# russellgeum/Digging-into-Self-Supervised-Monocular-Depth-Estimation

Hardware: AMD Instinct MI355X
Metric: images/sec training, KITTI 192x640 batch 12/GPU (higher is better)
Workload: dtype f32; 1 GPU; configs[1]: kitti_eigen_zhou-shaped 192x640, batch 12/GPU, ResNet18 depth + separate ResNet18 pose, frame_ids [0,-1,1], 4 scales, automask, Adam, fp32; global_batch=12, parallelism=dp1

## Files before the change

digging-into-self-supervised-monocular-depth-estimation_amd/csrc/thinconv_nhwc.hip:

```cpp
#include "nhwc_common.hpp"

namespace mdx {
namespace nhwc {

typedef float v4f __attribute__((ext_vector_type(4)));
constexpr int TW_WAVES = 4;

template <int CIN>
__global__ __launch_bounds__(64 * TW_WAVES) void thin_wgrad16_kernel(const float *__restrict__ x, const float *__restrict__ gy, int B, int h,
                                                                      int w, int quads_per_wave, float *__restrict__ part)
{
    constexpr int CH = CIN / 16, NT = 9 * CH;
    __shared__ float lds[TW_WAVES][256];
    const int lane = threadIdx.x & 63, wave = threadIdx.x >> 6;
    const int Hp = h + 2, Wp = w + 2, wq = w / 4;
    const long long nquads = (long long)B * h * wq;
    const long long q0 = ((long long)blockIdx.x * TW_WAVES + wave) * quads_per_wave;
    const long long q1 = q0 + quads_per_wave < nquads ? q0 + quads_per_wave : nquads;
    v4f acc[NT];
#pragma unroll
    for (int t = 0; t < NT; ++t) acc[t] = (v4f){0.f, 0.f, 0.f, 0.f};
    const int k = lane >> 4, j = lane & 15;
    if (q0 < q1) {
        int qx = (int)(q0 % wq);
        const long long row0 = q0 / wq;
        int i = (int)(row0 % h);
        const int b0 = (int)(row0 / h);
        const float *pg = gy + (size_t)q0 * 64 + lane;
        const float *px = x + (((size_t)b0 * Hp + i) * Wp + (size_t)qx * 4 + k) * CIN + j;
        auto load_b = [&](const float *xb, float (&bv)[NT]) {
#pragma unroll
            for (int ty = 0; ty < 3; ++ty)
#pragma unroll
                for (int tx = 0; tx < 3; ++tx)
#pragma unroll
                    for (int c = 0; c < CH; ++c) bv[(ty * 3 + tx) * CH + c] = xb[((size_t)ty * Wp + tx) * CIN + c * 16];
        };
        auto advance = [&]() {
            pg += 64;
            px += 4 * CIN;
            if (++qx == wq) {
                qx = 0;
                px += 2 * CIN;
                if (++i == h) { i = 0; px += (size_t)2 * Wp * CIN; }
            }
        };
        float a0 = *pg, b0v[NT];
        load_b(px, b0v);
        for (long long q = q0; q < q1; ++q) {
            float a1 = 0.f, b1v[NT];
            advance();
            if (q + 1 < q1) {
                a1 = *pg;
                load_b(px, b1v);
            } else {
#pragma unroll
                for (int t = 0; t < NT; ++t) b1v[t] = 0.f;
            }
#pragma unroll
            for (int t = 0; t < NT; ++t) acc[t] = __builtin_amdgcn_mfma_f32_16x16x4f32(a0, b0v[t], acc[t], 0, 0, 0);
            a0 = a1;
#pragma unroll
            for (int t = 0; t < NT; ++t) b0v[t] = b1v[t];
        }
    }
    float *dst = part + (size_t)blockIdx.x * NT * 256;
#pragma unroll
    for (int t = 0; t < NT; ++t) {
#pragma unroll
        for (int v = 0; v < 4; ++v) lds[wave][(4 * k + v) * 16 + j] = acc[t][v];
        __syncthreads();
        {
            const int r = threadIdx.x;
            float s = lds[0][r];
#pragma unroll
            for (int u = 1; u < TW_WAVES; ++u) s += lds[u][r];
            dst[t * 256 + r] = s;
        }
        __syncthreads();
    }
}

constexpr int TF_S = 64;
__global__ __launch_bounds__(16 * TF_S) void thin_wgrad16_finish_kernel(const float *__restrict__ part, int nblk, int CIN, long wso, long wsc,
                                                                        long wsy, long wsx, float *__restrict__ gw)
{
    __shared__ float lds[TF_S / 4][16];
    const int n = 9 * CIN * 16;
    const int cl = threadIdx.x % 16, sl = threadIdx.x / 16, e = blockIdx.x * 16 + cl;
    float s = 0.f;
    for (int i = sl; i < nblk; i += TF_S) s += (e < n) ? part[(size_t)i * n + e] : 0.f;
    s += __shfl_down(s, 32, 64);
    s += __shfl_down(s, 16, 64);
    if ((threadIdx.x & 63) < 16) lds[threadIdx.x >> 6][cl] = s;
    __syncthreads();
    if (threadIdx.x < 16 && e < n) {
        float tot = 0.f;
#pragma unroll
        for (int u = 0; u < TF_S / 4; ++u) tot += lds[u][cl];
        const int CH = CIN / 16;
        const int t = e >> 8, r = e & 255, co = r >> 4, cj = r & 15;
        const int tap = t / CH, ci = (t % CH) * 16 + cj;
        gw[co * wso + ci * wsc + (tap / 3) * wsy + (tap % 3) * wsx] = tot;
    }
}

struct ThinGeom { int blocks, quads_per_wave; };
static inline ThinGeom thin_geom(int B, int h, int w)
{
    const long long nquads = (long long)B * h * (w / 4);
    ThinGeom g;
    long long waves = 6144;
    if (waves * 48 > nquads) waves = (nquads + 47) / 48;
    if (waves < 1) waves = 1;
    g.quads_per_wave = (int)((nquads + waves - 1) / waves);
    g.blocks = (int)((nquads + (long long)g.quads_per_wave * TW_WAVES - 1) / ((long long)g.quads_per_wave * TW_WAVES));
    return g;
}

}
}

using namespace mdx;
using namespace mdx::nhwc;

static int thin_args_ok(int B, int Cin, int Cout, int h, int w)
{
    if (B <= 0 || h <= 0 || w <= 0 || w % 4 || Cout != 16 || (Cin != 16 && Cin != 32)) return MDX_ERR_BAD_SHAPE;
    if ((long long)B * (h + 2) * (w + 2) * Cin >= (1ll << 40)) return MDX_ERR_BAD_SHAPE;
    return MDX_OK;
}

MDX_EXPORT size_t mdx_thin_conv3x3_wgrad_workspace_bytes(int B, int Cin, int Cout, int h, int w)
{
    if (thin_args_ok(B, Cin, Cout, h, w)) return 0;
    return (size_t)thin_geom(B, h, w).blocks * 9 * Cin * 16 * sizeof(float);
}

MDX_EXPORT int mdx_thin_conv3x3_wgrad(const float *x, const float *gy, float *gweight, int64_t s_o, int64_t s_c, int64_t s_y, int64_t s_x,
                                      int B, int Cin, int Cout, int h, int w, void *workspace, size_t workspace_bytes, void *stream)
{
    if (!x || !gy || !gweight || !workspace) return MDX_ERR_NULL_POINTER;
    const int bad = thin_args_ok(B, Cin, Cout, h, w);
    if (bad) return bad;
    if (workspace_bytes < mdx_thin_conv3x3_wgrad_workspace_bytes(B, Cin, Cout, h, w)) return MDX_ERR_WORKSPACE;
    const ThinGeom g = thin_geom(B, h, w);
    float *part = (float *)workspace;
    hipStream_t st = (hipStream_t)stream;
    if (Cin == 16)
        hipLaunchKernelGGL((thin_wgrad16_kernel<16>), dim3(g.blocks), dim3(64 * TW_WAVES), 0, st, x, gy, B, h, w, g.quads_per_wave, part);
    else
        hipLaunchKernelGGL((thin_wgrad16_kernel<32>), dim3(g.blocks), dim3(64 * TW_WAVES), 0, st, x, gy, B, h, w, g.quads_per_wave, part);
    const int n = 9 * Cin * 16;
    hipLaunchKernelGGL(thin_wgrad16_finish_kernel, dim3((n + 15) / 16), dim3(16 * TF_S), 0, st, part, g.blocks, Cin, (long)s_o, (long)s_c,
                       (long)s_y, (long)s_x, gweight);
    return check_launch();
}
```

digging-into-self-supervised-monocular-depth-estimation_amd/mdx/functional.py:

```python
import ctypes as C

import torch

from . import _lib
from ._lib import api, ptr, stream, workspace


def _f32c(t, keep_format=False):
    if t is not None and t.dtype != torch.float32:
        t = t.float()
    if t is None or t.is_contiguous() or (keep_format and t.is_contiguous(memory_format=torch.channels_last)):
        return t
    return t.contiguous()


def _byref(struct):
    return C.byref(struct) if struct is not None else None


class _ComposeProjection(torch.autograd.Function):
    @staticmethod
    def forward(ctx, K, T):
        K, T = _f32c(K), _f32c(T)
        B = K.shape[0]
# ... 467 lines not shown
        cam, P = ctx.saved_tensors
        B, H, W, eps = ctx.dims
        ggrid = _f32c(ggrid)
        gcam = torch.empty_like(cam)
        gP = torch.empty_like(P)
        nws = api.mdx_project_workspace_bytes(B, H, W)
        ws = workspace(nws, cam.device)
        api.mdx_project_bwd(ptr(cam), ptr(P), ptr(ggrid), B, H, W, eps, ptr(gcam), ptr(gP),
                            ptr(ws, torch.uint8), nws, stream())
        return gcam, gP, None, None, None


def project(cam, P, H, W, eps=1e-7):
    return _Project.apply(cam, P, int(H), int(W), float(eps))


class _GridSampleBorder(torch.autograd.Function):
    @staticmethod
    def forward(ctx, img, grid):
        img, grid = _f32c(img), _f32c(grid)
        B, Cc, Hi, Wi = img.shape
        _, Ho, Wo, _ = grid.shape
        out = torch.empty(B, Cc, Ho, Wo, device=img.device, dtype=torch.float32)
        api.mdx_grid_sample_border_fwd(ptr(img), ptr(grid), B, Cc, Hi, Wi, Ho, Wo, ptr(out), stream())
        ctx.save_for_backward(img, grid)
        return out

    @staticmethod
    def backward(ctx, gout):
        img, grid = ctx.saved_tensors
        B, Cc, Hi, Wi = img.shape
        _, Ho, Wo, _ = grid.shape
        gout = _f32c(gout)
        ggrid = torch.empty_like(grid)
        gimg = torch.empty_like(img) if ctx.needs_input_grad[0] else None
        api.mdx_grid_sample_border_bwd(ptr(img), ptr(grid), ptr(gout), B, Cc, Hi, Wi, Ho, Wo, ptr(ggrid),
                                       ptr(gimg, optional=True), stream())
        return gimg, ggrid


def grid_sample_border(img, grid):
    return _GridSampleBorder.apply(img, grid)


class _ReprojectionLoss(torch.autograd.Function):
    @staticmethod
    def forward(ctx, pred, target):
        pred, target = _f32c(pred), _f32c(target)
        B, _, H, W = pred.shape
        out = torch.empty(B, 1, H, W, device=pred.device, dtype=torch.float32)
        api.mdx_reprojection_loss_fwd(ptr(pred), ptr(target), B, H, W, ptr(out), stream())
        ctx.save_for_backward(pred, target)
        return out

    @staticmethod
    def backward(ctx, gout):
        pred, target = ctx.saved_tensors
        B, _, H, W = pred.shape
        gout = _f32c(gout)
        gp = torch.empty_like(pred) if ctx.needs_input_grad[0] else None
        gt = torch.empty_like(pred) if ctx.needs_input_grad[1] else None
        if gp is None and gt is None:
            return None, None
        api.mdx_reprojection_loss_bwd(ptr(pred), ptr(target), ptr(gout), B, H, W, ptr(gp, optional=True),
                                      ptr(gt, optional=True), stream())
        return gp, gt


def reprojection_loss(pred, target):
    return _ReprojectionLoss.apply(pred, target)


class _Ssim(torch.autograd.Function):
    @staticmethod
    def forward(ctx, x, y):
        x, y = _f32c(x), _f32c(y)
        B, Cc, H, W = x.shape
        out = torch.empty_like(x)
        api.mdx_ssim_fwd(ptr(x), ptr(y), B * Cc, H, W, ptr(out), stream())
        ctx.save_for_backward(x, y)
        return out

    @staticmethod
    def backward(ctx, gout):
        x, y = ctx.saved_tensors
        B, Cc, H, W = x.shape
        gout = _f32c(gout)
        gx = torch.empty_like(x) if ctx.needs_input_grad[0] else None
        gy = torch.empty_like(x) if ctx.needs_input_grad[1] else None
        if gx is None and gy is None:
            return None, None
        api.mdx_ssim_bwd(ptr(x), ptr(y), ptr(gout), B * Cc, H, W, ptr(gx, optional=True), ptr(gy, optional=True),
                         stream())
        return gx, gy


def ssim(x, y):
    return _Ssim.apply(x, y)


def min_automask(ident, noise, reproj, automask=True, need_combined=False):
    reproj = _f32c(reproj)
    B, S, H, W = reproj.shape
    dev = reproj.device
    if automask:
        ident, noise = _f32c(ident), _f32c(noise)
    Cc = 2 * S if automask else S
    comb = torch.empty(B, Cc, H, W, device=dev, dtype=torch.float32) if need_combined else None
    to_opt = torch.empty(B, H, W, device=dev, dtype=torch.float32)
    idx = torch.empty(B, H, W, device=dev, dtype=torch.uint8)
    api.mdx_min_automask_fwd(ptr(ident, optional=True) if automask else None,
                             ptr(noise, optional=True) if automask else None, ptr(reproj), B, S, H, W,
                             int(automask), ptr(comb, optional=True), ptr(to_opt), ptr(idx, torch.uint8), stream())
    return to_opt, idx, comb


_DTYPE_CODE = {torch.float32: 0, torch.bfloat16: 1}
_CL = torch.channels_last


from .layout import is_channels_last


def _nhwc_ok(dtype, *channels):
    n = 4 if dtype == torch.float32 else 8
    return all(c % n == 0 for c in channels)


def _layout(x, what, *channels):
    if not x.is_cuda:
        raise _lib.MdxError("%s needs CUDA tensors (the HIP path has no CPU fallback), got %s" % (what, x.device))
    if x.dtype not in _DTYPE_CODE:
        raise _lib.MdxError("%s supports float32 / bfloat16, got %s" % (what, x.dtype))
    cl = is_channels_last(x) and _nhwc_ok(x.dtype, *channels)
    return _DTYPE_CODE[x.dtype], cl, (_CL if cl else torch.contiguous_format)


def _as(t, cl):
    if t is None:
        return None
    return t.contiguous(memory_format=_CL) if cl else t.contiguous()


def _cl_map(x, dtypes=_DTYPE_CODE):
    return x.is_cuda and x.dim() == 4 and x.dtype in dtypes and is_channels_last(x)


class _DecoderGlue(torch.autograd.Function):
    @staticmethod
    def forward(ctx, raw, skip, bias, elu, upsample, out_dtype):
        B, C1, h, w = raw.shape
        u = 2 if upsample else 1
        C2 = 0
        if skip is not None:
            if skip.dtype != raw.dtype or skip.shape[0] != B or tuple(skip.shape[2:]) != (u * h, u * w):
                raise _lib.MdxError("decoder_glue: skip %s %s does not match raw %s %s (x%d)"
                                    % (tuple(skip.shape), skip.dtype, tuple(raw.shape), raw.dtype, u))
            C2 = skip.shape[1]
        in_code, cl, fmt = _layout(raw, "decoder_glue", C1, C2)
        raw, skip, bias = _as(raw, cl), _as(skip, cl), _f32c(bias)
        if bias is not None and bias.shape != (C1,):
            raise _lib.MdxError("decoder_glue: bias %s for %d channels" % (tuple(bias.shape), C1))
        out = torch.empty(B, C1 + C2, u * h + 2, u * w + 2, device=raw.device, dtype=out_dtype, memory_format=fmt)
        fn = api.mdx_decoder_glue_nhwc_fwd if cl else api.mdx_decoder_glue_fwd
        fn(ptr(raw, raw.dtype, cl=cl), ptr(skip, raw.dtype, optional=True, cl=cl), ptr(bias, optional=True),
           ptr(out, out_dtype, cl=cl), B, C1, C2, h, w, int(upsample), int(elu), in_code, _DTYPE_CODE[out_dtype], stream())
        ctx.save_for_backward(raw, bias)
        ctx.meta = (C2, bool(elu), bool(upsample), out_dtype, cl, fmt)
        return out

    @staticmethod
    def backward(ctx, gout):
        raw, bias = ctx.saved_tensors
        C2, elu, upsample, out_dtype, cl, fmt = ctx.meta
        B, C1, h, w = raw.shape
        u = 2 if upsample else 1
        gout = _as(gout.to(out_dtype), cl)
        graw = torch.empty_like(raw)
        gskip = torch.empty(B, C2, u * h, u * w, device=raw.device, dtype=raw.dtype, memory_format=fmt) if C2 else None
        dbias = ws = None
        nws = 0
        code = _DTYPE_CODE[raw.dtype]
        if bias is not None:
            dbias = torch.empty(C1, device=raw.device, dtype=torch.float32)
            nws = (api.mdx_decoder_glue_nhwc_workspace_bytes(B, C1, h, w, code) if cl
                   else api.mdx_decoder_glue_workspace_bytes(B, C1, h, w))
            ws = workspace(nws, raw.device)
        fn = api.mdx_decoder_glue_nhwc_bwd if cl else api.mdx_decoder_glue_bwd
        fn(ptr(gout, out_dtype, cl=cl), ptr(raw, raw.dtype, cl=cl), ptr(bias, optional=True), ptr(graw, raw.dtype, cl=cl),
           ptr(gskip, raw.dtype, optional=True, cl=cl), ptr(dbias, optional=True), B, C1, C2, h, w, int(upsample), int(elu), code,
           _DTYPE_CODE[out_dtype], ptr(ws, torch.uint8, optional=True), nws, stream())
        return graw, gskip, dbias, None, None, None


def decoder_glue(raw, skip=None, elu=True, upsample=True, out_dtype=None, bias=None):
    out_dtype = out_dtype or raw.dtype
    if skip is not None and skip.dtype != raw.dtype:
        skip = skip.to(raw.dtype)
    return _DecoderGlue.apply(raw, skip, bias, bool(elu), bool(upsample), out_dtype)


class _BiasAct(torch.autograd.Function):
    @staticmethod
    def forward(ctx, x, bias, relu):
        B, Cc, H, W = x.shape
        x = _as(x, True)
        y = torch.empty_like(x)
        api.mdx_bias_act_nhwc_fwd(ptr(x, x.dtype, cl=True), ptr(_f32c(bias)), ptr(y, x.dtype, cl=True), B, Cc, H, W, int(relu),
                                  _DTYPE_CODE[x.dtype], stream())
        ctx.save_for_backward(y)
        ctx.meta = (bool(relu), bias.dtype)
        return y

    @staticmethod
    def backward(ctx, dy):
        (y,) = ctx.saved_tensors
        relu, bdt = ctx.meta
        B, Cc, H, W = y.shape
        code = _DTYPE_CODE[y.dtype]
        dy = _as(dy.to(y.dtype), True)
        dx = torch.empty_like(y)
        db = torch.empty(Cc, device=y.device, dtype=torch.float32)
        nws = api.mdx_bias_act_nhwc_workspace_bytes(B, Cc, H, W, code)
        ws = workspace(nws, y.device)
        api.mdx_bias_act_nhwc_bwd(ptr(dy, y.dtype, cl=True), ptr(y, y.dtype, cl=True), ptr(dx, y.dtype, cl=True), ptr(db), B, Cc,
                                  H, W, int(relu), code, ptr(ws, torch.uint8), nws, stream())
        return dx, db.to(bdt), None


def bias_act_ok(x):
    return _cl_map(x) and _nhwc_ok(x.dtype, x.shape[1])


def bias_act(x, bias, relu=True):
    if not bias_act_ok(x):
        raise _lib.MdxError("bias_act: needs a channels-last GPU map with whole 16-byte channel vectors, got %s %s" % (tuple(x.shape), x.dtype))
    return _BiasAct.apply(x, bias, bool(relu))


class _MeanBias(torch.autograd.Function):
    @staticmethod
    def forward(ctx, x, bias, scale):
        B, Cc, H, W = x.shape
        x = _as(x, True)
        out = torch.empty(B, Cc, device=x.device, dtype=torch.float32)
        api.mdx_mean_bias_nhwc_fwd(ptr(x, x.dtype, cl=True), ptr(_f32c(bias), optional=True), ptr(out), B, Cc, H, W, scale,
                                   _DTYPE_CODE[x.dtype], stream())
        ctx.meta = (tuple(x.shape), x.dtype, float(scale), None if bias is None else bias.dtype)
        return out

    @staticmethod
    def backward(ctx, g):
        (B, Cc, H, W), dt, scale, bdt = ctx.meta
        g = _f32c(g)
        dx = torch.empty((B, Cc, H, W), device=g.device, dtype=dt, memory_format=_CL)
        db = torch.empty(Cc, device=g.device, dtype=torch.float32) if bdt is not None else None
        api.mdx_mean_bias_nhwc_bwd(ptr(g), ptr(dx, dt, cl=True), ptr(db, optional=True), B, Cc, H, W, scale, _DTYPE_CODE[dt],
                                   stream())
        return dx, (db.to(bdt) if db is not None else None), None


def mean_bias_ok(x):
    return _cl_map(x)


def mean_bias(x, bias=None, scale=1.0):
    if not mean_bias_ok(x):
        raise _lib.MdxError("mean_bias: needs a channels-last GPU map, got %s %s" % (tuple(x.shape), x.dtype))
    return _MeanBias.apply(x, bias, float(scale))


class FrameStack(object):

    def __init__(self, blocks):
        self.blocks = [list(b) for b in blocks]

    def tensor(self):
        rows = [torch.cat(b, 1) if len(b) > 1 else b[0] for b in self.blocks]
        return torch.cat(rows, 0) if len(rows) > 1 else rows[0]

    def ok(self):
        fr = [t for b in self.blocks for t in b]
        first = fr[0]
        return (1 <= len(self.blocks) <= 2 and len({len(b) for b in self.blocks}) == 1 and 1 <= len(self.blocks[0]) <= 2
                and all(t.is_cuda and t.dtype == torch.float32 and t.dim() == 4 and t.shape == first.shape and t.shape[1] == 3
                        and t.is_contiguous() and not t.requires_grad for t in fr))


def encoder_input(stack, mean=0.45, std=0.225, dtype=torch.float32):
    if not stack.ok():
        raise _lib.MdxError("encoder_input: needs 1-2 blocks of 1-2 planar float32 [n,3,H,W] GPU frames that require no gradient")
    fr = [t for b in stack.blocks for t in b]
    n, _, H, W = fr[0].shape
    blocks, groups = len(stack.blocks), len(stack.blocks[0])
    out = torch.empty((blocks * n, 3 * groups, H, W), device=fr[0].device, dtype=dtype, memory_format=_CL)
    inv = float(torch.tensor(1.0, dtype=torch.float32) / torch.tensor(std, dtype=torch.float32))
    api.mdx_encoder_input_nhwc(_lib.ptr_array(fr), blocks, groups, n, H, W, mean, inv, ptr(out, dtype, cl=True),
                               _DTYPE_CODE[dtype], stream())
    return out


class _ThinConv3x3(torch.autograd.Function):
    ARGS = ([1, 1], [0, 0], [1, 1], False, [0, 0], 1)

    @staticmethod
    def forward(ctx, x, weight):
        ctx.save_for_backward(x, weight)
        return torch.ops.aten.convolution(x, weight, None, *_ThinConv3x3.ARGS)

    @staticmethod
    def backward(ctx, gy):
        x, weight = ctx.saved_tensors
        gx = gw = None
        if ctx.needs_input_grad[0]:
            gx = torch.ops.aten.convolution_backward(gy, x, weight, None, *_ThinConv3x3.ARGS, [True, False, False])[0]
        if ctx.needs_input_grad[1]:
            B, Cin, Hp, Wp = x.shape
            gy = _as(gy, True)
            gw = torch.empty_like(weight)
            nws = api.mdx_thin_conv3x3_wgrad_workspace_bytes(B, Cin, 16, Hp - 2, Wp - 2)
            ws = workspace(nws, x.device)
            api.mdx_thin_conv3x3_wgrad(ptr(x, cl=True), ptr(gy, cl=True), ptr(gw, cl="any"), gw.stride(0), gw.stride(1),
                                       gw.stride(2), gw.stride(3), B, Cin, 16, Hp - 2, Wp - 2, ptr(ws, torch.uint8), nws, stream())
        return gx, gw


def thin_conv_ok(x, weight):
    return (_cl_map(x, (torch.float32,)) and weight.dtype == torch.float32 and tuple(weight.shape) == (16, x.shape[1], 3, 3)
            and x.shape[1] in (16, 32) and x.shape[3] > 2 and (x.shape[3] - 2) % 4 == 0 and x.shape[2] > 2
            and (weight.is_contiguous() or weight.is_contiguous(memory_format=_CL)) and not torch.is_autocast_enabled())


def thin_conv3x3(x, weight):
    if not thin_conv_ok(x, weight):
        raise _lib.MdxError("thin_conv3x3: needs a float32 channels-last map with 16 or 32 channels and a [16,Cin,3,3] weight, got %s %s"
                            % (tuple(x.shape), tuple(weight.shape)))
    return _ThinConv3x3.apply(x, weight)


class _DispHead(torch.autograd.Function):
    @staticmethod
    def forward(ctx, x, weight, bias):
        B, Cc, Hp, Wp = x.shape
        x = _as(x, True)
        w32 = _f32c(weight, keep_format=True)
        disp = torch.empty(B, 1, Hp - 2, Wp - 2, device=x.device, dtype=torch.float32)
        _, sc, sy, sx = w32.stride()
        api.mdx_disp_head_nhwc_fwd(ptr(x, x.dtype, cl=True), ptr(w32, cl="any"), sc, sy, sx, ptr(_f32c(bias), optional=True),
                                   ptr(disp), B, Cc, Hp - 2, Wp - 2, _DTYPE_CODE[x.dtype], stream())
        ctx.save_for_backward(x, w32, disp)
        ctx.meta = (weight.dtype, None if bias is None else bias.dtype)
        return disp

    @staticmethod
    def backward(ctx, g):
        x, w32, disp = ctx.saved_tensors
        wdt, bdt = ctx.meta
        B, Cc, Hp, Wp = x.shape
        code = _DTYPE_CODE[x.dtype]
        g = _f32c(g)
        gx = torch.empty_like(x)
        gw = torch.empty_like(w32)
        gb = torch.empty(1, device=x.device, dtype=torch.float32) if bdt is not None else None
        nws = api.mdx_disp_head_nhwc_workspace_bytes(B, Cc, Hp - 2, Wp - 2, code)
        ws = workspace(nws, x.device)
        _, sc, sy, sx = w32.stride()
        api.mdx_disp_head_nhwc_bwd(ptr(x, x.dtype, cl=True), ptr(w32, cl="any"), sc, sy, sx, ptr(g), ptr(disp),
                                   ptr(gx, x.dtype, cl=True), ptr(gw, cl="any"), ptr(gb, optional=True), B, Cc,
                                   Hp - 2, Wp - 2, code, ptr(ws, torch.uint8), nws, stream())
        return gx, gw.to(wdt), (gb.to(bdt) if gb is not None else None)


def disp_head_ok(x, weight):
    if not _cl_map(x):
        return False
    n = 4
    lp = x.shape[1] // n
    return (tuple(weight.shape) == (1, x.shape[1], 3, 3) and x.shape[1] % n == 0 and 1 <= lp <= 64 and lp & (lp - 1) == 0
            and x.shape[2] > 2 and x.shape[3] > 2)


def disp_head(x, weight, bias=None):
    if not disp_head_ok(x, weight):
        raise _lib.MdxError("disp_head: needs a channels-last GPU map [B,C,h+2,w+2] with C a power of two from 4 to 256 "
                            "and a [1,C,3,3] weight; got x %s %s, weight %s" % (tuple(x.shape), x.dtype, tuple(weight.shape)))
    return _DispHead.apply(x, weight, bias)


class _MaxPool3s2(torch.autograd.Function):
    @staticmethod
    def forward(ctx, x, fork):
        B, Cc, H, W = x.shape
        code, cl, fmt = _layout(x, "maxpool3s2", Cc)
        x = _as(x, cl)
        Ho, Wo = (H - 1) // 2 + 1, (W - 1) // 2 + 1
        out = torch.empty(B, Cc, Ho, Wo, device=x.device, dtype=x.dtype, memory_format=fmt)
        arg = torch.empty(B, Cc, Ho, Wo, device=x.device, dtype=torch.uint8, memory_format=fmt)
        if cl:
            api.mdx_maxpool3s2_nhwc_fwd(ptr(x, x.dtype, cl=True), ptr(out, x.dtype, cl=True),
                                        ptr(arg, torch.uint8, cl=True), B, Cc, H, W, code, stream())
        else:
            api.mdx_maxpool3s2_fwd(ptr(x, x.dtype), ptr(out, x.dtype), ptr(arg, torch.uint8), B * Cc, H, W, code,
                                   stream())
        ctx.save_for_backward(arg)
        ctx.meta = (H, W, x.dtype, cl, fmt)
        ctx.set_materialize_grads(False)
        return (out, out.view_as(out)) if fork else out

    @staticmethod
    def backward(ctx, gout, gout2=None):
        (arg,) = ctx.saved_tensors
        H, W, dtype, cl, fmt = ctx.meta
        B, Cc = arg.shape[:2]
        gout, gout2 = _two_grads(gout, gout2, dtype, cl, fused_add=cl)
        if gout is None:
            return None, None
        gin = torch.empty(B, Cc, H, W, device=gout.device, dtype=dtype, memory_format=fmt)
        if cl:
            api.mdx_maxpool3s2_nhwc_bwd(ptr(gout, dtype, cl=True), ptr(gout2, dtype, optional=True, cl=True),
                                        ptr(arg, torch.uint8, cl=True), ptr(gin, dtype, cl=True), B, Cc, H, W,
                                        _DTYPE_CODE[dtype], stream())
        else:
            api.mdx_maxpool3s2_bwd(ptr(gout, dtype), ptr(arg, torch.uint8), ptr(gin, dtype), B * Cc, H, W,
                                   _DTYPE_CODE[dtype], stream())
        return gin, None


def _two_grads(g1, g2, dtype, cl, fused_add):
    gs = [_as(g.to(dtype), cl) for g in (g1, g2) if g is not None]
    if not gs:
        return None, None
    if len(gs) == 2 and not fused_add:
        gs = [gs[0] + gs[1]]
    return gs[0], (gs[1] if len(gs) == 2 else None)


def maxpool3s2(x, fork=False):
    return _MaxPool3s2.apply(x, bool(fork))


def _residual(what, res, x):
    if res is not None and (res.shape != x.shape or res.dtype != x.dtype):
        raise _lib.MdxError("%s: residual %s %s does not match x %s %s" % (what, tuple(res.shape), res.dtype, tuple(x.shape), x.dtype))
    return res


class _BnAct(torch.autograd.Function):

    @staticmethod
    def forward(ctx, x, res, weight, bias, running_mean, running_var, eps, momentum, relu, groups, fork):
        B, Cc, H, W = x.shape
        code, cl, _ = _layout(x, "bn_act", Cc)
        if B % groups:
            raise _lib.MdxError("bn_act: batch %d is not divisible into %d groups" % (B, groups))
        x, res = _as(x, cl), _as(_residual("bn_act", res, x), cl)
        weight, bias = _f32c(weight), _f32c(bias)
        y = torch.empty_like(x)
        save_mean = torch.empty(groups, Cc, device=x.device, dtype=torch.float32)
        save_invstd = torch.empty(groups, Cc, device=x.device, dtype=torch.float32)
        Bg = B // groups
        nws = api.mdx_bn_nhwc_workspace_bytes(Bg, Cc, H, W, groups, code) if cl else api.mdx_bn_workspace_bytes(Bg, Cc, H, W)
        ws = workspace(nws, x.device)
        fn = api.mdx_bn_act_nhwc_fwd if cl else api.mdx_bn_act_fwd
        fn(ptr(x, x.dtype, cl=cl), ptr(res, x.dtype, optional=True, cl=cl), ptr(weight), ptr(bias),
           ptr(running_mean, optional=True), ptr(running_var, optional=True), ptr(y, x.dtype, cl=cl), ptr(save_mean),
           ptr(save_invstd), Bg, Cc, H, W, groups, eps, momentum, int(relu), code, ptr(ws, torch.uint8), nws, stream())
        mask_from_x = cl and bool(relu) and res is None and x.dtype == torch.float32
        ctx.save_for_backward(x, bias if mask_from_x else y, weight, save_mean, save_invstd)
        ctx.meta = (bool(relu), res is not None, groups, cl, mask_from_x)
        ctx.mark_non_differentiable(*[t for t in (running_mean, running_var) if t is not None])
        ctx.set_materialize_grads(False)
        return (y, y.view_as(y)) if fork else y

    @staticmethod
    def backward(ctx, dy, dy2=None):
        x, y, weight, save_mean, save_invstd = ctx.saved_tensors
        relu, has_res, groups, cl, mask_from_x = ctx.meta
        bias = None
        if mask_from_x:
            y, bias = None, y
        dy, dy2 = _two_grads(dy, dy2, x.dtype, cl, fused_add=cl)
        if dy is None:
            return (None,) * 11
        B, Cc, H, W = x.shape
        Bg = B // groups
        code = _DTYPE_CODE[x.dtype]
        dx = torch.empty_like(x)
        dres = torch.empty_like(x) if has_res else None
        dgamma = torch.empty(Cc, device=x.device, dtype=torch.float32)
        dbeta = torch.empty(Cc, device=x.device, dtype=torch.float32)
        nws = api.mdx_bn_nhwc_workspace_bytes(Bg, Cc, H, W, groups, code) if cl else api.mdx_bn_workspace_bytes(Bg, Cc, H, W)
        ws = workspace(nws, x.device)
        if cl:
            api.mdx_bn_act_nhwc_bwd(
                ptr(dy, x.dtype, cl=True), ptr(dy2, x.dtype, optional=True, cl=True), ptr(y, x.dtype, optional=True, cl=True),
                ptr(x, x.dtype, cl=True), ptr(weight), ptr(bias, optional=True), ptr(save_mean), ptr(save_invstd),
                ptr(dx, x.dtype, cl=True), ptr(dres, x.dtype, optional=True, cl=True), ptr(dgamma), ptr(dbeta), Bg, Cc, H, W,
                groups, int(relu), code, ptr(ws, torch.uint8), nws, stream())
        else:
            api.mdx_bn_act_bwd(
                ptr(dy, x.dtype), ptr(y, x.dtype), ptr(x, x.dtype), ptr(weight), ptr(save_mean), ptr(save_invstd),
                ptr(dx, x.dtype), ptr(dres, x.dtype, optional=True), ptr(dgamma), ptr(dbeta), Bg, Cc, H, W, groups,
                int(relu), code, ptr(ws, torch.uint8), nws, stream())
        return (dx, dres, dgamma, dbeta) + (None,) * 7


def bn_act(x, weight, bias, running_mean, running_var, eps=1e-5, momentum=0.1, residual=None, relu=True, groups=1,
           fork=False):
    return _BnAct.apply(x, residual, weight, bias, running_mean, running_var, float(eps), float(momentum), bool(relu),
                        int(groups), bool(fork))


def bn_act_infer(x, weight, bias, running_mean, running_var, eps=1e-5, residual=None, relu=True, fork=False):
    B, Cc, H, W = x.shape
    code, cl, _ = _layout(x, "bn_act_infer", Cc)
    x, residual = _as(x, cl), _as(_residual("bn_act_infer", residual, x), cl)
    y = torch.empty_like(x)
    fn = api.mdx_bn_act_nhwc_infer if cl else api.mdx_bn_act_infer
    fn(ptr(x, x.dtype, cl=cl), ptr(residual, x.dtype, optional=True, cl=cl), ptr(_f32c(weight)),
       ptr(_f32c(bias)), ptr(_f32c(running_mean)), ptr(_f32c(running_var)), ptr(y, x.dtype, cl=cl), B, Cc, H, W, float(eps),
       int(bool(relu)), code, stream())
    return (y, y.view_as(y)) if fork else y


class _Param2Matrix(torch.autograd.Function):
    @staticmethod
    def forward(ctx, axisangle, translation, invert):
        aa, tr = _f32c(axisangle).reshape(-1, 3), _f32c(translation).reshape(-1, 3)
        N = aa.shape[0]
        if tr.shape[0] != N:
            raise _lib.MdxError("param2matrix: %d rotations, %d translations" % (N, tr.shape[0]))
        M = torch.empty(N, 4, 4, device=aa.device, dtype=torch.float32)
        api.mdx_param2matrix_fwd(ptr(aa), ptr(tr), N, int(invert), ptr(M), stream())
        ctx.save_for_backward(aa, tr)
        ctx.meta = (bool(invert), axisangle.shape, translation.shape)
        return M

    @staticmethod
    def backward(ctx, gM):
        aa, tr = ctx.saved_tensors
        invert, sa, st = ctx.meta
        gM = _f32c(gM)
        gaa, gtr = torch.empty_like(aa), torch.empty_like(tr)
        api.mdx_param2matrix_bwd(ptr(aa), ptr(tr), ptr(gM), aa.shape[0], int(invert), ptr(gaa), ptr(gtr),
                                 stream())
        return gaa.reshape(sa), gtr.reshape(st), None


def param2matrix(axisangle, translation, invert=False):
    return _Param2Matrix.apply(axisangle, translation, bool(invert))


class _PoseProjection(torch.autograd.Function):
    @staticmethod
    def forward(ctx, raw, K, B, row0, frame, invert):
        raw, K = _f32c(raw), _f32c(K)
        M, F = raw.shape[0], raw.shape[1]
        S = len(row0)
        T = torch.empty(S, B, 4, 4, device=raw.device, dtype=torch.float32)
        P = torch.empty(S, B, 3, 4, device=raw.device, dtype=torch.float32)
        sel = tuple((C.c_int32 * S)(*[int(v) for v in a]) for a in (row0, frame, invert))
        api.mdx_pose_projection_fwd(ptr(raw), M, F, ptr(K), B, S, *sel, ptr(T), ptr(P), stream())
        ctx.save_for_backward(raw, K)
        ctx.meta = (B, [int(v) for v in row0], [int(v) for v in frame], [int(v) for v in invert])
        return T, P

    @staticmethod
    def backward(ctx, gT, gP):
        raw, K = ctx.saved_tensors
        B, row0, frame, invert = ctx.meta
        M, F = raw.shape[0], raw.shape[1]
        S = len(row0)
        graw = torch.empty_like(raw)
        sel = tuple((C.c_int32 * S)(*a) for a in (row0, frame, invert))
        api.mdx_pose_projection_bwd(ptr(raw), M, F, ptr(K), B, S, *sel,
                                    ptr(_f32c(gP), optional=True), ptr(_f32c(gT), optional=True), ptr(graw), stream())
        return graw, None, None, None, None, None


def pose_projection(raw, K, row0, frame, invert):
    if K.requires_grad:
        raise _lib.MdxError("pose_projection: K must not require a gradient (use param2matrix + compose_projection)")
    B = K.shape[0]
    return _PoseProjection.apply(raw.reshape(raw.shape[0], raw.shape[1], 6), K, B, list(row0), list(frame), list(invert))


def depth_monitor(pred, gt, window, min_depth=1e-3, max_depth=80.0):
    pred, gt = _f32c(pred), _f32c(gt)
    B, _, h, w = pred.shape
    _, _, gh, gw = gt.shape
    r0, r1, c0, c1 = (int(v) for v in window)
    out = torch.empty(8, device=pred.device, dtype=torch.float32)
    nws = api.mdx_depth_monitor_workspace_bytes(B, r0, r1, c0, c1)
    ws = workspace(nws, pred.device)
    api.mdx_depth_monitor(ptr(pred), B, h, w, ptr(gt), gh, gw, r0, r1, c0, c1, min_depth, max_depth, ptr(out),
                          ptr(ws, torch.uint8), nws, stream())
    return out
```

include/mdx.h:

```cpp
#ifndef MDX_H
#define MDX_H

#include <stddef.h>
#include <stdint.h>

#ifdef __cplusplus
extern "C" {
#endif

#define MDX_VERSION 510
#define MDX_MAX_SRC 4
#define MDX_MAX_SCALES 4

typedef enum mdx_status {
    MDX_OK = 0,
    MDX_ERR_BAD_SHAPE = -1,
    MDX_ERR_NULL_POINTER = -2,
    MDX_ERR_WORKSPACE = -3,
    MDX_ERR_LAUNCH = -4,
    MDX_ERR_UNSUPPORTED = -5,
    MDX_ERR_MISALIGNED = -6
} mdx_status;

#define MDX_FLAG_AUTOMASK 1u
#define MDX_FLAG_UPSAMPLE_PREMUL 2u
#define MDX_FLAG_FASTDIV_W 4u
#define MDX_FLAG_FASTDIV_H 8u

typedef struct mdx_desc {
    int32_t B, H, W;
    int32_t h, w;
    int32_t S;
    uint32_t flags;
    float disp_a, disp_b;
} mdx_desc;

typedef struct mdx_sources {
    const float *img[MDX_MAX_SRC];
} mdx_sources;

int mdx_desc_init(mdx_desc *d, int B, int H, int W, int h, int w, int S, int automask,
                  double min_depth, double max_depth);

int mdx_version(void);
const char *mdx_status_string(int status);


int mdx_compose_projection(const float *K, const float *T, int B, float *P, void *stream);

int mdx_identity_loss(const mdx_desc *d, const float *target, const mdx_sources *src, float *ident,
                      void *stream);

size_t mdx_photometric_workspace_bytes(const mdx_desc *d);

int mdx_photometric_fwd(const mdx_desc *d, const float *disp, const float *target,
                        const mdx_sources *src, const float *invK, const float *P,
                        const float *ident, const float *noise, uint8_t *idx, float *loss_sum,
                        float *to_opt, float *depth, float *warp, float *reproj, float *coef,
                        void *workspace, size_t workspace_bytes, void *stream);

typedef struct mdx_timing { void *start, *stop; } mdx_timing;
void *mdx_event_create(void);
void mdx_event_destroy(void *event);
int mdx_event_elapsed_us(void *start, void *stop, float *us);

int mdx_photometric_fwd_timed(const mdx_desc *d, const float *disp, const float *target,
                              const mdx_sources *src, const float *invK, const float *P,
                              const float *ident, const float *noise, uint8_t *idx, float *loss_sum,
                              float *to_opt, float *depth, float *warp, float *reproj, float *coef,
                              void *workspace, size_t workspace_bytes, void *stream, const mdx_timing *t);

int mdx_photometric_bwd(const mdx_desc *d, const float *disp, const float *target,
                        const mdx_sources *src, const float *invK, const float *P,
                        const uint8_t *idx, const float *warp, const float *coef, float g_const,
                        const float *g_dev, float *gdisp, float *gP, void *workspace, size_t workspace_bytes,
                        void *stream);
int mdx_photometric_bwd_timed(const mdx_desc *d, const float *disp, const float *target,
                        const mdx_sources *src, const float *invK, const float *P,
                        const uint8_t *idx, const float *warp, const float *coef, float g_const,
                        const float *g_dev, float *gdisp, float *gP, void *workspace, size_t workspace_bytes,
                        void *stream, const mdx_timing *t);

typedef struct mdx_train_desc {
    int32_t B, H, W;
    int32_t S;
    int32_t nscales;
    uint32_t flags;
    float disp_a, disp_b;
    int32_t h[MDX_MAX_SCALES], w[MDX_MAX_SCALES];
    int32_t rows_per_chunk;
} mdx_train_desc;

int mdx_train_desc_init(mdx_train_desc *d, int B, int H, int W, int S, int nscales, const int32_t *h,
                        const int32_t *w, int automask, double min_depth, double max_depth, int rows_per_chunk);
size_t mdx_photometric_train_workspace_bytes(const mdx_train_desc *d);

int mdx_photometric_train(const mdx_train_desc *d, const float *const *disp, const float *target,
                          const mdx_sources *src, const float *invK, const float *const *P, const float *ident,
                          const float *const *noise, uint8_t *const *idx, float *loss_sum, float *const *gdisp,
                          float *gP, float *depth0, float *const *to_opt, void *workspace, size_t workspace_bytes,
                          void *stream, const mdx_timing *t);

int mdx_photometric_prologue(const mdx_train_desc *d, const float *target, const mdx_sources *src,
                             const float *const *noise, unsigned long long *rng_state, int advance_rng,
                             float *ident, float *tstat, float *const *bidfi, void *stream);

int mdx_photometric_train_pre(const mdx_train_desc *d, const float *const *disp, const float *target,
                              const mdx_sources *src, const float *invK, const float *const *P,
                              const float *tstat, const float *const *bidfi, unsigned long long *rng_state,
                              uint8_t *const *idx, float *loss_sum, float *const *gdisp, float *gP, float *depth0,
                              float *const *to_opt, void *workspace, size_t workspace_bytes, void *stream,
                              const mdx_timing *t);

size_t mdx_smooth_workspace_bytes(int B, int h, int w);
int mdx_smooth_loss(int B, int h, int w, const float *disp, const float *color, int normalize, float *loss,
                    float *gdisp, void *workspace, size_t workspace_bytes, void *stream);

size_t mdx_smooth_multi_workspace_bytes(int nscales, int B, const int32_t *h, const int32_t *w);
int mdx_smooth_loss_multi(int nscales, int B, const int32_t *h, const int32_t *w, const float *const *disp,
                          const float *const *color, int normalize, float *loss, float *const *gdisp,
                          void *workspace, size_t workspace_bytes, void *stream);

int mdx_loss_total_fwd(int nscales, const float *sums, const float *smooth, const int32_t *scale, int64_t pixels,
                       double disp_smoothness, float *total, void *stream);
int mdx_loss_total_bwd(int nscales, const float *g_total, const int32_t *scale, int64_t pixels, double disp_smoothness,
                       const float *const *gd_photo, const float *const *gd_smooth, const int64_t *count,
                       float *const *gdisp, const float *gP, int nP, int per_scale_P, float *gP_out, void *stream);

int mdx_adam_max_tensors(void);
int mdx_adam_chunk(void);
size_t mdx_adam_table_entry_bytes(void);
int mdx_adam_step(const void *table, int first, int count, const float *const *grads, const void *blockmap, int nblocks,
                  const float *lr_ptr, double lr, double beta1, double beta2, double eps, void *stream);

size_t mdx_adam_guard_record_bytes(void);
size_t mdx_adam_guard_partials_bytes(int nblocks);
int mdx_adam_grad_sumsq(const void *table, int first, int count, const float *const *grads, const void *blockmap, int nblocks,
                        double *partials, void *stream);
int mdx_adam_guard_finish(const void *table, int ntensors, const double *partials, int npartials, double max_grad_norm,
                          int skip_nonfinite, void *record, void *stream);
int mdx_adam_step_guarded(const void *table, int first, int count, const float *const *grads, const void *blockmap, int nblocks,
                          const float *lr_ptr, double lr, double beta1, double beta2, double eps, const void *record, void *stream);


int mdx_interpolate_bilinear_fwd(const float *x, int BC, int h, int w, float *out, int H, int W,
                                 void *stream);
int mdx_interpolate_bilinear_bwd(const float *gout, int BC, int H, int W, float *gin, int h, int w,
                                 void *stream);

int mdx_disparity2depth_fwd(const float *disp, size_t n, double min_depth, double max_depth,
                            float *sd, float *depth, void *stream);
int mdx_disparity2depth_bwd(const float *disp, const float *gsd, const float *gdepth, size_t n,
                            double min_depth, double max_depth, float *gdisp, void *stream);

int mdx_backproject_fwd(const float *depth, const float *invK, int B, int H, int W, float *cam,
                        void *stream);
int mdx_backproject_bwd(const float *gcam, const float *invK, int B, int H, int W, float *gdepth,
                        void *stream);

size_t mdx_project_workspace_bytes(int B, int H, int W);
int mdx_project_fwd(const float *cam, const float *P, int B, int H, int W, float eps, float *grid,
                    void *stream);
int mdx_project_bwd(const float *cam, const float *P, const float *ggrid, int B, int H, int W,
                    float eps, float *gcam, float *gP, void *workspace, size_t workspace_bytes,
                    void *stream);

int mdx_grid_sample_border_fwd(const float *img, const float *grid, int B, int C, int Hi, int Wi,
                               int Ho, int Wo, float *out, void *stream);
int mdx_grid_sample_border_bwd(const float *img, const float *grid, const float *gout, int B, int C,
                               int Hi, int Wi, int Ho, int Wo, float *ggrid, float *gimg,
                               void *stream);

int mdx_reprojection_loss_fwd(const float *pred, const float *target, int B, int H, int W,
                              float *out, void *stream);
int mdx_reprojection_loss_bwd(const float *pred, const float *target, const float *gout, int B,
                              int H, int W, float *gpred, float *gtarget, void *stream);
int mdx_ssim_fwd(const float *x, const float *y, int BC, int H, int W, float *out, void *stream);
int mdx_ssim_bwd(const float *x, const float *y, const float *gout, int BC, int H, int W, float *gx, float *gy,
                 void *stream);

int mdx_min_automask_fwd(const float *ident, const float *noise, const float *reproj, int B, int S,
                         int H, int W, int automask, float *combined, float *to_opt, uint8_t *idx,
                         void *stream);

int mdx_param2matrix_fwd(const float *axisangle, const float *translation, int N, int invert, float *M, void *stream);
int mdx_param2matrix_bwd(const float *axisangle, const float *translation, const float *gM, int N, int invert,
                         float *gaxisangle, float *gtranslation, void *stream);

int mdx_pose_projection_fwd(const float *raw, int M, int F, const float *K, int B, int S, const int32_t *row0,
                            const int32_t *frame, const int32_t *invert, float *T, float *P, void *stream);
int mdx_pose_projection_bwd(const float *raw, int M, int F, const float *K, int B, int S, const int32_t *row0,
                            const int32_t *frame, const int32_t *invert, const float *gP, const float *gT, float *graw,
                            void *stream);


int mdx_decoder_glue_fwd(const void *raw, const void *skip, const float *bias, void *out, int B, int C1, int C2, int h,
                         int w, int upsample, int elu, int in_dtype, int out_dtype, void *stream);
size_t mdx_decoder_glue_workspace_bytes(int B, int C1, int h, int w);
int mdx_decoder_glue_bwd(const void *gout, const void *raw, const float *bias, void *graw, void *gskip, float *dbias,
                         int B, int C1, int C2, int h, int w, int upsample, int elu, int in_dtype, int out_dtype,
                         void *workspace, size_t workspace_bytes, void *stream);

int mdx_maxpool3s2_fwd(const void *in, void *out, uint8_t *arg, int BC, int H, int W, int dtype, void *stream);
int mdx_maxpool3s2_bwd(const void *gout, const uint8_t *arg, void *gin, int BC, int H, int W, int dtype, void *stream);

size_t mdx_bn_workspace_bytes(int B, int C, int H, int W);
int mdx_bn_act_fwd(const void *x, const void *res, const float *gamma, const float *beta, float *run_mean,
                   float *run_var, void *y, float *save_mean, float *save_invstd, int B, int C, int H, int W,
                   int groups, float eps, float momentum, int relu, int dtype, void *workspace, size_t workspace_bytes,
                   void *stream);
int mdx_bn_act_bwd(const void *dy, const void *y, const void *x, const float *gamma, const float *save_mean,
                   const float *save_invstd, void *dx, void *dres, float *dgamma, float *dbeta, int B, int C, int H,
                   int W, int groups, int relu, int dtype, void *workspace, size_t workspace_bytes, void *stream);

int mdx_bn_act_infer(const void *x, const void *res, const float *gamma, const float *beta, const float *run_mean,
                     const float *run_var, void *y, int B, int C, int H, int W, float eps, int relu, int dtype,
                     void *stream);
int mdx_bn_act_nhwc_infer(const void *x, const void *res, const float *gamma, const float *beta, const float *run_mean,
                          const float *run_var, void *y, int B, int C, int H, int W, float eps, int relu, int dtype,
                          void *stream);

size_t mdx_bn_nhwc_workspace_bytes(int B, int C, int H, int W, int groups, int dtype);
int mdx_bn_act_nhwc_fwd(const void *x, const void *res, const float *gamma, const float *beta, float *run_mean,
                        float *run_var, void *y, float *save_mean, float *save_invstd, int B, int C, int H, int W,
                        int groups, float eps, float momentum, int relu, int dtype, void *workspace,
                        size_t workspace_bytes, void *stream);
int mdx_bn_act_nhwc_bwd(const void *dy, const void *dy2, const void *y, const void *x, const float *gamma,
                        const float *beta, const float *save_mean, const float *save_invstd, void *dx, void *dres, float *dgamma,
                        float *dbeta, int B, int C, int H, int W, int groups, int relu, int dtype, void *workspace,
                        size_t workspace_bytes, void *stream);
size_t mdx_bias_act_nhwc_workspace_bytes(int B, int C, int H, int W, int dtype);
int mdx_bias_act_nhwc_fwd(const void *x, const float *bias, void *y, int B, int C, int H, int W, int relu, int dtype, void *stream);
int mdx_bias_act_nhwc_bwd(const void *dy, const void *y, void *dx, float *dbias, int B, int C, int H, int W, int relu, int dtype,
                          void *workspace, size_t workspace_bytes, void *stream);
int mdx_mean_bias_nhwc_fwd(const void *x, const float *bias, float *out, int B, int C, int H, int W, float scale, int dtype,
                           void *stream);
int mdx_mean_bias_nhwc_bwd(const float *gout, void *dx, float *dbias, int B, int C, int H, int W, float scale, int dtype,
                           void *stream);

int mdx_encoder_input_nhwc(const float *const *src, int blocks, int groups, int n, int H, int W, float mean, float inv_std,
                           void *out, int dtype, void *stream);

size_t mdx_thin_conv3x3_wgrad_workspace_bytes(int B, int Cin, int Cout, int h, int w);
int mdx_thin_conv3x3_wgrad(const float *x, const float *gy, float *gweight, int64_t s_o, int64_t s_c, int64_t s_y, int64_t s_x, int B,
                           int Cin, int Cout, int h, int w, void *workspace, size_t workspace_bytes, void *stream);

size_t mdx_disp_head_nhwc_workspace_bytes(int B, int C, int h, int w, int dtype);
int mdx_disp_head_nhwc_fwd(const void *x, const float *weight, int64_t w_stride_c, int64_t w_stride_ky, int64_t w_stride_kx,
                           const float *bias, float *disp, int B, int C, int h, int w, int dtype, void *stream);
int mdx_disp_head_nhwc_bwd(const void *x, const float *weight, int64_t w_stride_c, int64_t w_stride_ky, int64_t w_stride_kx,
                           const float *gdisp, const float *disp, void *gx, float *gweight, float *gbias, int B, int C, int h,
                           int w, int dtype, void *workspace, size_t workspace_bytes, void *stream);
int mdx_decoder_glue_nhwc_fwd(const void *raw, const void *skip, const float *bias, void *out, int B, int C1, int C2,
                              int h, int w, int upsample, int elu, int in_dtype, int out_dtype, void *stream);
size_t mdx_decoder_glue_nhwc_workspace_bytes(int B, int C1, int h, int w, int in_dtype);
int mdx_decoder_glue_nhwc_bwd(const void *gout, const void *raw, const float *bias, void *graw, void *gskip,
                              float *dbias, int B, int C1, int C2, int h, int w, int upsample, int elu, int in_dtype,
                              int out_dtype, void *workspace, size_t workspace_bytes, void *stream);
int mdx_maxpool3s2_nhwc_fwd(const void *in, void *out, uint8_t *arg, int B, int C, int H, int W, int dtype,
                            void *stream);
int mdx_maxpool3s2_nhwc_bwd(const void *gout, const void *gout2, const uint8_t *arg, void *gin, int B, int C, int H,
                            int W, int dtype, void *stream);

size_t mdx_depth_monitor_workspace_bytes(int B, int r0, int r1, int c0, int c1);
int mdx_depth_monitor(const float *pred, int B, int h, int w, const float *gt, int gh, int gw, int r0, int r1, int c0,
                      int c1, float min_depth, float max_depth, float *out, void *workspace, size_t workspace_bytes,
                      void *stream);

#define MDX_IMG_JOBS 72
#define MDX_JITTER_JOBS 56
#define MDX_JITTER_PARTIALS 128

int mdx_resample_ksize(int in_size, int out_size);
int mdx_resample_plan(int in_size, int out_size, int *bounds, int *kk);
int mdx_resample_plan_cols(int in_size, int out_size, int *lead, int *row, int *table);

typedef struct mdx_resample_job {
    const uint8_t *src;
    const int *xbounds, *xkk;
    const int *ybounds, *ykk;
    uint8_t *inter;
    uint8_t *dst_u8;
    float *dst_f32;
    int in_h, in_w, in_stride, flip;
    int out_h, out_w, xksize, yksize;
    const int *xkc;
    int xkc_lead, xkc_row;
} mdx_resample_job;
int mdx_resample_lanczos_u8(const mdx_resample_job *jobs, int njobs, void *stream);

typedef struct mdx_jitter_job {
    const uint8_t *src;
    float *dst_f32;
    uint8_t *dst_u8;
    unsigned long long *lsum;
    int h, w;
    int order[4];
    int hue_shift;
    float brightness, contrast, saturation;
} mdx_jitter_job;
int mdx_color_jitter_u8(const mdx_jitter_job *jobs, int njobs, void *stream);

int mdx_color_convert_u8(int mode, const uint8_t *src, uint8_t *dst, size_t npix, void *stream);

int mdx_to_tensor_u8(const uint8_t *src, float *dst, size_t n, void *stream);

#ifdef __cplusplus
}
#endif
#endif
```

Baseline: 827.2 images/s.

## Add MFMA-based NHWC forward and dgrad kernels for thin 16-channel 3x3 convs

```diff
diff --git a/digging-into-self-supervised-monocular-depth-estimation_amd/csrc/thinconv_nhwc.hip b/digging-into-self-supervised-monocular-depth-estimation_amd/csrc/thinconv_nhwc.hip
--- a/digging-into-self-supervised-monocular-depth-estimation_amd/csrc/thinconv_nhwc.hip
+++ b/digging-into-self-supervised-monocular-depth-estimation_amd/csrc/thinconv_nhwc.hip
@@ -118,6 +118,131 @@
     return g;
 }
 
+constexpr int TC_WAVES = 4;
+constexpr int TC_MIN_ROWS = 12;
+
+template <int KC, int NC, bool DG>
+__device__ __forceinline__ void thin_conv_rows(const float *__restrict__ src, const float *__restrict__ wt, long wso, long wsc, long wsy,
+                                               long wsx, float *__restrict__ dst, int B, int Hs, int Ws, int rows_per_wave)
+{
+    constexpr int KCH = KC / 16, NT = NC / 16, P = DG ? 2 : 0, NL = 3 * KCH;
+    const int lane = threadIdx.x & 63, wave = threadIdx.x >> 6;
+    const int i = lane & 15, g = lane >> 4;
+    const int Ho = Hs + 2 * P - 2, Wo = Ws + 2 * P - 2, nt = (Wo + 15) / 16;
+    const long long R = (long long)B * Ho, units = R * nt;
+    const long long u0 = ((long long)blockIdx.x * TC_WAVES + wave) * rows_per_wave;
+    const long long u1 = u0 + rows_per_wave < units ? u0 + rows_per_wave : units;
+    if (u0 >= u1) return;
+    float wr[9][KCH][NT][4];
+#pragma unroll
+    for (int ty = 0; ty < 3; ++ty)
+#pragma unroll
+        for (int tx = 0; tx < 3; ++tx)
+#pragma unroll
+            for (int c = 0; c < KCH; ++c)
+#pragma unroll
+                for (int n = 0; n < NT; ++n)
+#pragma unroll
+                    for (int j = 0; j < 4; ++j) {
+                        const int kc = c * 16 + 4 * g + j, nc = n * 16 + i;
+                        wr[ty * 3 + tx][c][n][j] = DG ? wt[kc * wso + nc * wsc + (2 - ty) * wsy + (2 - tx) * wsx]
+                                                      : wt[nc * wso + kc * wsc + ty * wsy + tx * wsx];
+                    }
+    int t = (int)(u0 / R);
+    const long long rr = u0 % R;
+    int b = (int)(rr / Ho), r = (int)(rr % Ho);
+    auto load_row = [&](int rs, v4f (&v)[NL]) {
+        const int row = rs - P;
+        const bool row_ok = !DG || (row >= 0 && row < Hs);
+        const float *p = src + ((size_t)b * Hs + (row_ok ? row : 0)) * Ws * KC + 4 * g;
+#pragma unroll
+        for (int tx = 0; tx < 3; ++tx) {
+            const int col = t * 16 + i + tx - P;
+            const bool ok = row_ok && col >= 0 && col < Ws;
+#pragma unroll
+            for (int c = 0; c < KCH; ++c)
+                v[tx * KCH + c] = ok ? *(const v4f *)(p + (size_t)col * KC + c * 16) : (v4f){0.f, 0.f, 0.f, 0.f};
+        }
+    };
+    v4f win[3][NL], nxt[NL];
+    bool fresh = true;
+    for (long long u = u0; u < u1; ++u) {
+        if (fresh) {
+            load_row(r, win[0]);
+            load_row(r + 1, win[1]);
+            load_row(r + 2, win[2]);
+        } else {
+#pragma unroll
+            for (int l = 0; l < NL; ++l) win[2][l] = nxt[l];
+        }
+        const bool more = u + 1 < u1 && r + 1 < Ho;
+        if (more) load_row(r + 3, nxt);
+        v4f acc[NT][2];
+#pragma unroll
+        for (int n = 0; n < NT; ++n) acc[n][0] = acc[n][1] = (v4f){0.f, 0.f, 0.f, 0.f};
+#pragma unroll
+        for (int ty = 0; ty < 3; ++ty)
+#pragma unroll
+            for (int tx = 0; tx < 3; ++tx)
+#pragma unroll
+                for (int c = 0; c < KCH; ++c)
+#pragma unroll
+                    for (int j = 0; j < 4; ++j)
+#pragma unroll
+                        for (int n = 0; n < NT; ++n)
+                            acc[n][j & 1] = __builtin_amdgcn_mfma_f32_16x16x4f32(wr[ty * 3 + tx][c][n][j], win[ty][tx * KCH + c][j],
+                                                                                 acc[n][j & 1], 0, 0, 0);
+        const int col = t * 16 + i;
+        if (col < Wo) {
+            float *q = dst + (((size_t)b * Ho + r) * Wo + col) * NC + 4 * g;
+#pragma unroll
+            for (int n = 0; n < NT; ++n) *(v4f *)(q + n * 16) = acc[n][0] + acc[n][1];
+        }
+        if (more) {
+#pragma unroll
+            for (int l = 0; l < NL; ++l) { win[0][l] = win[1][l]; win[1][l] = win[2][l]; }
+            ++r;
+            fresh = false;
+        } else {
+            fresh = true;
+            if (++r == Ho) {
+                r = 0;
+                if (++b == B) { b = 0; ++t; }
+            }
+        }
+    }
+}
+
+template <int CIN>
+__global__ __launch_bounds__(64 * TC_WAVES) void thin_fwd16_kernel(const float *__restrict__ x, const float *__restrict__ wt, long wso, long wsc,
+                                                                    long wsy, long wsx, float *__restrict__ y, int B, int h, int w,
+                                                                    int rows_per_wave)
+{
+    thin_conv_rows<CIN, 16, false>(x, wt, wso, wsc, wsy, wsx, y, B, h + 2, w + 2, rows_per_wave);
+}
+
+template <int CIN>
+__global__ __launch_bounds__(64 * TC_WAVES) void thin_dgrad16_kernel(const float *__restrict__ gy, const float *__restrict__ wt, long wso,
+                                                                      long wsc, long wsy, long wsx, float *__restrict__ gx, int B, int h, int w,
+                                                                      int rows_per_wave)
+{
+    thin_conv_rows<16, CIN, true>(gy, wt, wso, wsc, wsy, wsx, gx, B, h, w, rows_per_wave);
+}
+
+struct ThinConvGeom { int blocks, rows_per_wave; };
+static inline ThinConvGeom thin_conv_geom(int B, int Ho, int Wo)
+{
+    const long long units = (long long)B * Ho * ((Wo + 15) / 16);
+    long long per_simd = (units + 1024ll * TC_MIN_ROWS / 2) / (1024ll * TC_MIN_ROWS);
+    per_simd = per_simd < 1 ? 1 : per_simd > 4 ? 4 : per_simd;
+    long long rows = (units + 1024 * per_simd - 1) / (1024 * per_simd);
+    if (rows < TC_MIN_ROWS) rows = TC_MIN_ROWS;
+    ThinConvGeom q;
+    q.rows_per_wave = (int)rows;
+    q.blocks = (int)((units + rows * TC_WAVES - 1) / (rows * TC_WAVES));
+    return q;
+}
+
 }
 }
 
@@ -156,3 +281,37 @@
                        (long)s_y, (long)s_x, gweight);
     return check_launch();
 }
+
+MDX_EXPORT int mdx_thin_conv3x3_fwd(const float *x, const float *weight, int64_t s_o, int64_t s_c, int64_t s_y, int64_t s_x, float *y, int B,
+                                    int Cin, int Cout, int h, int w, void *stream)
+{
+    if (!x || !weight || !y) return MDX_ERR_NULL_POINTER;
+    const int bad = thin_args_ok(B, Cin, Cout, h, w);
+    if (bad) return bad;
+    const ThinConvGeom q = thin_conv_geom(B, h, w);
+    hipStream_t st = (hipStream_t)stream;
+    if (Cin == 16)
+        hipLaunchKernelGGL((thin_fwd16_kernel<16>), dim3(q.blocks), dim3(64 * TC_WAVES), 0, st, x, weight, (long)s_o, (long)s_c, (long)s_y,
+                           (long)s_x, y, B, h, w, q.rows_per_wave);
+    else
+        hipLaunchKernelGGL((thin_fwd16_kernel<32>), dim3(q.blocks), dim3(64 * TC_WAVES), 0, st, x, weight, (long)s_o, (long)s_c, (long)s_y,
+                           (long)s_x, y, B, h, w, q.rows_per_wave);
+    return check_launch();
+}
+
+MDX_EXPORT int mdx_thin_conv3x3_dgrad(const float *gy, const float *weight, int64_t s_o, int64_t s_c, int64_t s_y, int64_t s_x, float *gx,
+                                      int B, int Cin, int Cout, int h, int w, void *stream)
+{
+    if (!gy || !weight || !gx) return MDX_ERR_NULL_POINTER;
+    const int bad = thin_args_ok(B, Cin, Cout, h, w);
+    if (bad) return bad;
+    const ThinConvGeom q = thin_conv_geom(B, h + 2, w + 2);
+    hipStream_t st = (hipStream_t)stream;
+    if (Cin == 16)
+        hipLaunchKernelGGL((thin_dgrad16_kernel<16>), dim3(q.blocks), dim3(64 * TC_WAVES), 0, st, gy, weight, (long)s_o, (long)s_c,
+                           (long)s_y, (long)s_x, gx, B, h, w, q.rows_per_wave);
+    else
+        hipLaunchKernelGGL((thin_dgrad16_kernel<32>), dim3(q.blocks), dim3(64 * TC_WAVES), 0, st, gy, weight, (long)s_o, (long)s_c,
+                           (long)s_y, (long)s_x, gx, B, h, w, q.rows_per_wave);
+    return check_launch();
+}
diff --git a/digging-into-self-supervised-monocular-depth-estimation_amd/mdx/functional.py b/digging-into-self-supervised-monocular-depth-estimation_amd/mdx/functional.py
--- a/digging-into-self-supervised-monocular-depth-estimation_amd/mdx/functional.py
+++ b/digging-into-self-supervised-monocular-depth-estimation_amd/mdx/functional.py
@@ -793,21 +793,33 @@
 
 class _ThinConv3x3(torch.autograd.Function):
     ARGS = ([1, 1], [0, 0], [1, 1], False, [0, 0], 1)
+    native_fwd = True
+    native_dgrad = True
 
     @staticmethod
     def forward(ctx, x, weight):
         ctx.save_for_backward(x, weight)
-        return torch.ops.aten.convolution(x, weight, None, *_ThinConv3x3.ARGS)
+        if not _ThinConv3x3.native_fwd:
+            return torch.ops.aten.convolution(x, weight, None, *_ThinConv3x3.ARGS)
+        B, Cin, Hp, Wp = x.shape
+        y = torch.empty((B, 16, Hp - 2, Wp - 2), device=x.device, dtype=torch.float32, memory_format=_CL)
+        api.mdx_thin_conv3x3_fwd(ptr(x, cl=True), ptr(weight, cl="any"), weight.stride(0), weight.stride(1), weight.stride(2),
+                                 weight.stride(3), ptr(y, cl=True), B, Cin, 16, Hp - 2, Wp - 2, stream())
+        return y
 
     @staticmethod
     def backward(ctx, gy):
         x, weight = ctx.saved_tensors
+        B, Cin, Hp, Wp = x.shape
         gx = gw = None
-        if ctx.needs_input_grad[0]:
+        if ctx.needs_input_grad[0] and not _ThinConv3x3.native_dgrad:
             gx = torch.ops.aten.convolution_backward(gy, x, weight, None, *_ThinConv3x3.ARGS, [True, False, False])[0]
+        gy = _as(gy, True)
+        if ctx.needs_input_grad[0] and _ThinConv3x3.native_dgrad:
+            gx = torch.empty_like(x)
+            api.mdx_thin_conv3x3_dgrad(ptr(gy, cl=True), ptr(weight, cl="any"), weight.stride(0), weight.stride(1), weight.stride(2),
+                                       weight.stride(3), ptr(gx, cl=True), B, Cin, 16, Hp - 2, Wp - 2, stream())
         if ctx.needs_input_grad[1]:
-            B, Cin, Hp, Wp = x.shape
-            gy = _as(gy, True)
             gw = torch.empty_like(weight)
             nws = api.mdx_thin_conv3x3_wgrad_workspace_bytes(B, Cin, 16, Hp - 2, Wp - 2)
             ws = workspace(nws, x.device)
diff --git a/include/mdx.h b/include/mdx.h
--- a/include/mdx.h
+++ b/include/mdx.h
@@ -245,6 +245,11 @@
 int mdx_thin_conv3x3_wgrad(const float *x, const float *gy, float *gweight, int64_t s_o, int64_t s_c, int64_t s_y, int64_t s_x, int B,
                            int Cin, int Cout, int h, int w, void *workspace, size_t workspace_bytes, void *stream);
 
+int mdx_thin_conv3x3_fwd(const float *x, const float *weight, int64_t s_o, int64_t s_c, int64_t s_y, int64_t s_x, float *y, int B, int Cin,
+                         int Cout, int h, int w, void *stream);
+int mdx_thin_conv3x3_dgrad(const float *gy, const float *weight, int64_t s_o, int64_t s_c, int64_t s_y, int64_t s_x, float *gx, int B,
+                           int Cin, int Cout, int h, int w, void *stream);
+
 size_t mdx_disp_head_nhwc_workspace_bytes(int B, int C, int h, int w, int dtype);
 int mdx_disp_head_nhwc_fwd(const void *x, const float *weight, int64_t w_stride_c, int64_t w_stride_ky, int64_t w_stride_kx,
                            const float *bias, float *disp, int B, int C, int h, int w, int dtype, void *stream);
```

After: 831.8 images/s, median of 6. About the same (+0.6%).
